# prs-eth/Marigold

Measured on AMD Instinct MI355X. Metric: depth maps/sec @768x768, ens=10, 10 DDIM steps, higher is better.
Workload: dtype bf16; 1 GPU; marigold-depth-v1-1 architecture (SD-v2 UNet 865.9M + AutoencoderKL), 768x768, ensemble_size=10, 10 DDIM steps (trailing, zero-SNR, v-prediction), seeded synthetic weights; members_per_gpu=10, parallelism=member-parallel x1, hipgraph=False, maps_in_flight=2

## Files before the change

include/marigold_hip.h:

```cpp
#ifndef MARIGOLD_HIP_H
#define MARIGOLD_HIP_H

#include <stdint.h>

#ifdef __cplusplus
extern "C" {
#endif

#define MG_ABI_VERSION 4

enum mg_op_kind {
  MG_OP_IGEMM = 1,
  MG_OP_GN_STATS = 2,
  MG_OP_GN_FINALIZE = 3,
  MG_OP_GN_APPLY = 4,
  MG_OP_GN_SLAB = 9,
  MG_OP_ROWGEMM = 10,
  MG_OP_FLASH_ATTN64 = 6,
  MG_OP_FLASH_ATTN512 = 11,
  MG_OP_SOFTMAX_ROWS = 7,
  MG_OP_SCHED_STEP = 12,
  MG_OP_LINEAR_SMALL_M = 13,
  MG_OP_LATENT_1X1 = 14,
  MG_OP_POST_NCHW = 15,
// ... 675 lines not shown
  const float* conv_b[5];
  const float* lin_w[5];
} mg_lpips_net;
long long mg_lpips_workspace_bytes(int H, int W);
int mg_eval_iid_lpips(const mg_lpips_net* net, const float* pred, const float* gt, const uint8_t* mask_or_null, int H, int W,
                      int up_to_scale, int gamma_mode, double* out8, void* eval_ws, void* act_ws, long long act_ws_bytes, void* stream);

int mg_rgb_prepare(const uint8_t* src, int hwc, int Hin, int Win, void* dst, int out16, int Hout, int Wout, int mode, int reciprocal,
                   float* tmp_or_null, void* stream);
int mg_normals_visualize(const float* pred, int H, int W, uint8_t* out_hwc, void* stream);
int mg_depth_visualize(const float* depth, const uint8_t* lut256x3_or_null, int64_t n, float* clipped_out_or_null,
                       uint16_t* u16_out_or_null, uint8_t* picture_out_or_null, void* stream);
int mg_normals_finish(const float* pred, int H, int W, float* clipped_out_or_null, uint8_t* picture_out_or_null, void* stream);

int mg_randn(uint64_t seed, uint64_t stream_id, int64_t offset, int64_t n, void* dst, int out16, void* stream);
int mg_resize(const void* src, void* dst, float* tmp_or_null, int planes, int Hin, int Win, int Hout, int Wout, int mode, int u8,
              void* stream);
int mg_colorize(const float* depth, const uint8_t* lut256x3, uint8_t* out_hwc, int64_t n, float min_depth, float max_depth, void* stream);
int mg_iid_visualize(const float* pred, uint8_t* out_hwc, float* workspace_or_null, int n_targets, int H, int W, int linear_bits,
                     int up_to_scale_bits, void* stream);

int mg_ens_align_cost_grad(int E, const double* s, const double* t, const double* mean, const double* C,
                           double* cost, double* gs, double* gt);
int mg_bfgs_minimize(int (*fn)(void* user, int n, const double* x, double* f, double* g), void* user, int n, double* x,
                     double gtol, int maxiter, double* fval, int* nit, int* nfev, int* status);
int mg_ens_align_minimize(const mg_op* reg_op, void* stream, int E, int affine, int reduction, double lam, const double* mean,
                          const double* C, float* st_host, const float* mm_host, double* x, double gtol, int maxiter,
                          double* fval, int* nit, int* nfev, int* status);

int mg_clock_probe(void* stream, int zero_operands, double* mhz, double* tflops);

int mg_debug_read_workspace(void* host_dst, long long bytes);

void* mg_event_create(void);
int mg_event_record(void* ev, void* stream);
int mg_event_elapsed_ms(void* start, void* stop, float* ms);
void mg_event_destroy(void* ev);

#ifdef __cplusplus
}
#endif
#endif
```

marigold_amd/_lib.py:

```python
import ctypes
import os

_HERE = os.path.dirname(os.path.abspath(__file__))
LIB_PATH = os.environ.get("MARIGOLD_HIP_LIB") or os.path.join(_HERE, "libmarigold_hip.so")
ABI_VERSION = 4

OP_IGEMM, OP_GN_STATS, OP_GN_FINALIZE, OP_GN_APPLY = 1, 2, 3, 4
OP_FLASH_ATTN64, OP_SOFTMAX_ROWS = 6, 7
OP_GN_SLAB = 9
OP_ROWGEMM = 10
OP_FLASH_ATTN512 = 11
RG_BF16, RG_GEGLU, RG_QKV, RG_XATTN = 0, 1, 2, 3
OP_SCHED_STEP = 12
OP_LINEAR_SMALL_M, OP_LATENT_1X1, OP_POST_NCHW, OP_IM2COL_SMALL = 13, 14, 15, 16
OP_CONV3X3 = 17
OP_CONV3X3_HEAD = 18
OP_ENS_DEPTH_STATS, OP_ENS_DEPTH_MEDIAN, OP_ENS_DEPTH_NORM, OP_ENS_NORMALS = 20, 21, 22, 23
OP_RESIZE = 24
OP_COLORIZE = 25
OP_EVAL_DEPTH_LS, OP_EVAL_DEPTH_METRICS, OP_EVAL_NORMALS = 26, 27, 28
EVAL_WS_BYTES = 128 * 1024
EVAL_ALIGN = {None: 0, "least_square": 1, "least_square_disparity": 2}
OP_MEMSET, OP_COPY = 30, 31
OP_IIDSCORE_PREP, OP_IIDSCORE_PSNR, OP_IIDSCORE_SSIM = 32, 33, 34
# ... 136 lines not shown
        p=("pred", "gt", "mask", "sums", "out", "scratch"))),
    OP_EVAL_NORMALS: ("EVAL_NORMALS", dict(
        i=("masked",),
        p=("pred", "gt", "out", "err", "ws"),
        l=("hw",))),
    OP_MEMSET: ("MEMSET", dict(
        i=("value",),
        p=("dst",),
        l=("bytes",))),
    OP_COPY: ("COPY", dict(
        p=("src", "dst"),
        l=("bytes",))),
    OP_IIDSCORE_PREP: ("IIDSCORE_PREP", dict(
        i=("h", "w", "gamma"),
        p=("pred", "gt", "mask", "out", "ws"))),
    OP_IIDSCORE_PSNR: ("IIDSCORE_PSNR", dict(
        i=("h", "w", "gamma", "up_to_scale", "write_psnr"),
        p=("pred", "gt", "mask", "out", "ws"))),
    OP_IIDSCORE_SSIM: ("IIDSCORE_SSIM", dict(
        i=("h", "w", "gamma", "up_to_scale"),
        p=("pred", "gt", "mask", "out", "ws"))),
    OP_IID_VIS: ("IID_VIS", dict(
        i=("n", "h", "w", "linear_bits", "up_to_scale_bits"),
        p=("pred", "out", "ws"))),
}

OP_NAMES = {v: k[3:].lower() for k, v in list(globals().items()) if k.startswith("OP_")}

EXPORTS = [
    "mg_abi_version", "mg_operand_bits", "mg_last_error", "mg_init", "mg_geglu_interleave", "mg_device_info", "mg_launch",
    "mg_program_create", "mg_program_num_ops", "mg_program_run", "mg_program_validate", "mg_program_run_range",
    "mg_program_capture", "mg_program_profile", "mg_program_destroy", "mg_conv2d_igemm", "mg_conv3x3", "mg_conv3x3_gn_slots", "mg_flash4w_plan_test",
    "mg_sched_step", "mg_ensemble_normals", "mg_ens_align_cost_grad", "mg_bfgs_minimize", "mg_ens_align_minimize", "mg_event_create", "mg_event_record",
    "mg_event_elapsed_ms", "mg_event_destroy", "mg_clock_probe", "mg_debug_read_workspace",
    "mg_model_load", "mg_model_destroy", "mg_model_info", "mg_model_device_bytes", "mg_model_validate", "mg_model_vae_encode",
    "mg_model_denoise", "mg_model_vae_decode", "mg_ensemble_depth", "mg_eval_depth", "mg_eval_normals", "mg_eval_iid",
    "mg_rgb_prepare", "mg_normals_visualize",
    "mg_randn", "mg_resize", "mg_colorize", "mg_iid_visualize", "mg_model_predict",
    "mg_ensemble_iid", "mg_model_predict_iid",
    "mg_depth_visualize", "mg_normals_finish", "mg_model_predict_out",
    "mg_lpips_workspace_bytes", "mg_eval_iid_lpips",
]


class MgPredictOpts(ctypes.Structure):
    _fields_ = [("scale_invariant", ctypes.c_int), ("shift_invariant", ctypes.c_int), ("reduction", ctypes.c_int), ("max_iter", ctypes.c_int),
                ("max_res", ctypes.c_int), ("normals_reduction", ctypes.c_int), ("regularizer_strength", ctypes.c_double), ("tol", ctypes.c_double)]

    def __init__(self, scale_invariant=1, shift_invariant=1, reduction=0, max_iter=50, max_res=1024, normals_reduction=0,
                 regularizer_strength=0.02, tol=1e-6):
        super().__init__(scale_invariant, shift_invariant, reduction, max_iter, max_res, normals_reduction, regularizer_strength, tol)


class MgIidOpts(ctypes.Structure):
    _fields_ = [("reduction", ctypes.c_int), ("linear_bits", ctypes.c_int), ("up_to_scale_bits", ctypes.c_int), ("out_h", ctypes.c_int),
                ("out_w", ctypes.c_int), ("out_mode", ctypes.c_int)]


class MgOutputOpts(ctypes.Structure):
    _fields_ = [("out_h", ctypes.c_int), ("out_w", ctypes.c_int), ("out_mode", ctypes.c_int), ("lut256x3", ctypes.c_void_p)]


class MgLpipsNet(ctypes.Structure):
    _fields_ = [("conv_w", ctypes.c_void_p * 5), ("conv_b", ctypes.c_void_p * 5), ("lin_w", ctypes.c_void_p * 5)]


class MgOp(ctypes.Structure):
# ... 23 lines not shown
    missing = [s for s in EXPORTS if not hasattr(lib, s)]
    if missing:
        raise MarigoldHipError(f"{path} lacks ABI symbols: {missing}")
    lib.mg_last_error.restype = ctypes.c_char_p
    lib.mg_launch.argtypes = [ctypes.POINTER(MgOp), ctypes.c_void_p]
    lib.mg_geglu_interleave.restype = ctypes.c_int
    lib.mg_conv2d_igemm.argtypes = [ctypes.POINTER(MgOp), ctypes.c_void_p]
    lib.mg_conv3x3.argtypes = [ctypes.POINTER(MgOp), ctypes.c_void_p]
    lib.mg_conv3x3_gn_slots.argtypes = [ctypes.POINTER(MgOp)]
    lib.mg_conv3x3_gn_slots.restype = ctypes.c_int
    lib.mg_flash4w_plan_test.argtypes = [ctypes.c_int] * 4 + [ctypes.c_longlong, ctypes.c_int, ctypes.POINTER(ctypes.c_int), ctypes.POINTER(ctypes.c_uint)]
    lib.mg_program_create.restype = ctypes.c_void_p
    lib.mg_program_create.argtypes = [ctypes.POINTER(MgOp), ctypes.c_int]
    lib.mg_program_num_ops.argtypes = [ctypes.c_void_p]
    lib.mg_ens_align_cost_grad.argtypes = [ctypes.c_int] + [ctypes.c_void_p] * 7
    lib.mg_bfgs_minimize.argtypes = [ctypes.c_void_p, ctypes.c_void_p, ctypes.c_int, ctypes.c_void_p, ctypes.c_double, ctypes.c_int,
                                     ctypes.c_void_p, ctypes.c_void_p, ctypes.c_void_p, ctypes.c_void_p]
    lib.mg_ens_align_minimize.argtypes = [ctypes.c_void_p, ctypes.c_void_p, ctypes.c_int, ctypes.c_int, ctypes.c_int, ctypes.c_double,
                                          ctypes.c_void_p, ctypes.c_void_p, ctypes.c_void_p, ctypes.c_void_p, ctypes.c_void_p,
                                          ctypes.c_double, ctypes.c_int, ctypes.c_void_p, ctypes.c_void_p, ctypes.c_void_p, ctypes.c_void_p]
    lib.mg_program_run.argtypes = [ctypes.c_void_p, ctypes.c_void_p]
    lib.mg_program_validate.argtypes = [ctypes.c_void_p]
    lib.mg_program_run_range.argtypes = [ctypes.c_void_p, ctypes.c_int, ctypes.c_int, ctypes.c_void_p]
    lib.mg_program_capture.argtypes = [ctypes.c_void_p, ctypes.c_void_p]
    lib.mg_program_profile.argtypes = [ctypes.c_void_p, ctypes.c_void_p, ctypes.POINTER(ctypes.c_float)]
    lib.mg_program_destroy.argtypes = [ctypes.c_void_p]
    lib.mg_program_destroy.restype = None
    lib.mg_sched_step.argtypes = [ctypes.c_void_p] * 4 + [ctypes.c_int64] + [ctypes.c_float] * 3 + [ctypes.c_void_p]
    lib.mg_ensemble_normals.argtypes = [ctypes.c_void_p] * 3 + [ctypes.c_int, ctypes.c_int64, ctypes.c_int, ctypes.c_void_p]
    lib.mg_device_info.argtypes = [ctypes.POINTER(ctypes.c_int), ctypes.POINTER(ctypes.c_int),
                                   ctypes.POINTER(ctypes.c_int64), ctypes.c_char_p, ctypes.c_int]
    lib.mg_clock_probe.argtypes = [ctypes.c_void_p, ctypes.c_int, ctypes.POINTER(ctypes.c_double), ctypes.POINTER(ctypes.c_double)]
    lib.mg_debug_read_workspace.argtypes = [ctypes.c_void_p, ctypes.c_longlong]
    lib.mg_model_load.restype = ctypes.c_void_p
    lib.mg_model_load.argtypes = [ctypes.c_char_p, ctypes.c_int]
    lib.mg_model_destroy.argtypes = [ctypes.c_void_p]
    lib.mg_model_destroy.restype = None
    lib.mg_model_info.argtypes = [ctypes.c_void_p, ctypes.POINTER(ctypes.c_int)]
    lib.mg_model_device_bytes.argtypes = [ctypes.c_void_p]
    lib.mg_model_device_bytes.restype = ctypes.c_longlong
    lib.mg_model_validate.argtypes = [ctypes.c_void_p]
    lib.mg_model_vae_encode.argtypes = [ctypes.c_void_p] * 4
    lib.mg_model_denoise.argtypes = [ctypes.c_void_p] * 5
    lib.mg_model_vae_decode.argtypes = [ctypes.c_void_p] * 4
    lib.mg_ensemble_depth.argtypes = [ctypes.c_void_p, ctypes.c_int, ctypes.c_int, ctypes.c_int, ctypes.c_int, ctypes.c_int, ctypes.c_int, ctypes.c_double,
                                      ctypes.c_int, ctypes.c_double, ctypes.c_int, ctypes.c_void_p, ctypes.c_void_p, ctypes.c_void_p, ctypes.c_void_p]
    lib.mg_eval_depth.argtypes = [ctypes.c_void_p] * 3 + [ctypes.c_int] * 4 + [ctypes.c_double] * 2 + [ctypes.c_void_p] * 3
    lib.mg_eval_normals.argtypes = [ctypes.c_void_p] * 2 + [ctypes.c_int64, ctypes.c_int] + [ctypes.c_void_p] * 4
    lib.mg_eval_iid.argtypes = [ctypes.c_void_p] * 3 + [ctypes.c_int] * 5 + [ctypes.c_void_p] * 3
    lib.mg_lpips_workspace_bytes.argtypes = [ctypes.c_int, ctypes.c_int]
    lib.mg_lpips_workspace_bytes.restype = ctypes.c_longlong
    lib.mg_eval_iid_lpips.argtypes = [ctypes.POINTER(MgLpipsNet)] + [ctypes.c_void_p] * 3 + [ctypes.c_int] * 4 + [ctypes.c_void_p] * 3 + \
        [ctypes.c_longlong, ctypes.c_void_p]
    lib.mg_rgb_prepare.argtypes = [ctypes.c_void_p] + [ctypes.c_int] * 3 + [ctypes.c_void_p] + [ctypes.c_int] * 5 + [ctypes.c_void_p] * 2
    lib.mg_normals_visualize.argtypes = [ctypes.c_void_p, ctypes.c_int, ctypes.c_int, ctypes.c_void_p, ctypes.c_void_p]
    lib.mg_randn.argtypes = [ctypes.c_uint64, ctypes.c_uint64, ctypes.c_int64, ctypes.c_int64, ctypes.c_void_p, ctypes.c_int, ctypes.c_void_p]
    lib.mg_resize.argtypes = [ctypes.c_void_p] * 3 + [ctypes.c_int] * 7 + [ctypes.c_void_p]
    lib.mg_colorize.argtypes = [ctypes.c_void_p] * 3 + [ctypes.c_int64, ctypes.c_float, ctypes.c_float, ctypes.c_void_p]
    lib.mg_iid_visualize.argtypes = [ctypes.c_void_p] * 3 + [ctypes.c_int] * 5 + [ctypes.c_void_p]
    lib.mg_model_predict.argtypes = [ctypes.c_void_p] * 2 + [ctypes.c_int] * 5 + [ctypes.c_uint64, ctypes.POINTER(MgPredictOpts)] + [ctypes.c_void_p] * 4
    lib.mg_ensemble_iid.argtypes = [ctypes.c_void_p, ctypes.c_int, ctypes.c_int64, ctypes.c_int, ctypes.c_void_p, ctypes.c_void_p, ctypes.c_void_p]
    lib.mg_model_predict_iid.argtypes = [ctypes.c_void_p] * 2 + [ctypes.c_int] * 5 + [ctypes.c_uint64, ctypes.POINTER(MgIidOpts)] + [ctypes.c_void_p] * 4
    lib.mg_depth_visualize.argtypes = [ctypes.c_void_p] * 2 + [ctypes.c_int64] + [ctypes.c_void_p] * 4
    lib.mg_normals_finish.argtypes = [ctypes.c_void_p, ctypes.c_int, ctypes.c_int] + [ctypes.c_void_p] * 3
    lib.mg_model_predict_out.argtypes = [ctypes.c_void_p] * 2 + [ctypes.c_int] * 5 + [ctypes.c_uint64, ctypes.POINTER(MgPredictOpts),
                                                                                       ctypes.POINTER(MgOutputOpts)] + [ctypes.c_void_p] * 6
# ... 31 lines not shown
```

marigold_amd/csrc/common.h:

```cpp
#pragma once
#include <hip/hip_runtime.h>
#include <stdint.h>

#include <type_traits>
#include "../../include/marigold_hip.h"

constexpr bool MG_F16 = MG_OPERAND_F16_BUILD != 0;
typedef uint16_t bf16_t;
typedef std::conditional_t<MG_F16, _Float16, __bf16> mg_op16_t;
typedef __attribute__((ext_vector_type(8))) mg_op16_t bf16x8;
typedef __attribute__((ext_vector_type(2))) mg_op16_t mg_bf16x2_t;
typedef __attribute__((ext_vector_type(2))) float mg_f32x2_t;
typedef __attribute__((ext_vector_type(16))) float f32x16;
typedef __attribute__((ext_vector_type(4))) float f32x4;

#define GLOBAL_AS __attribute__((address_space(1)))
#define LDS_AS __attribute__((address_space(3)))

#if MG_OPERAND_F16_BUILD
#define MG_MFMA32_ASM "v_mfma_f32_32x32x16_f16"
#define MG_MFMA16_ASM "v_mfma_f32_16x16x32_f16"
#define MG_CVT_PK_ASM "v_cvt_pk_f16_f32"
#else
#define MG_MFMA32_ASM "v_mfma_f32_32x32x16_bf16"
// ... 107 lines not shown
}

struct mg_fastdiv {
  uint32_t m, l;
};
inline mg_fastdiv mg_make_fastdiv(long long d) {
  mg_fastdiv f;
  uint32_t l = 0;
  while ((1ull << l) < (unsigned long long)d) ++l;
  f.l = l;
  f.m = (uint32_t)(((1ull << (31 + l)) + (unsigned long long)d - 1) / (unsigned long long)d);
  return f;
}
__device__ __forceinline__ int fdiv(int x, const mg_fastdiv f) { return (int)(__umulhi((uint32_t)x << 1, f.m) >> f.l); }

constexpr bool MG_HANDOFF_FENCES = MG_HANDOFF_FENCES_BUILD != 0;
__device__ __forceinline__ void mg_handoff_release() {
  if constexpr (MG_HANDOFF_FENCES) {
    __builtin_amdgcn_fence(__ATOMIC_RELEASE, "agent");
    asm volatile("s_waitcnt vmcnt(0)" ::: "memory");
  }
}
__device__ __forceinline__ void mg_handoff_acquire() {
  if constexpr (MG_HANDOFF_FENCES) __builtin_amdgcn_fence(__ATOMIC_ACQUIRE, "agent");
}

#define MG_ZERO_BYTES (128 * 1024)
extern void* g_zero_page;
extern thread_local bool g_dry_run;
#define MG_SPLITK_WS_BYTES (64ll * 1024 * 1024)
#define MG_LN_COUNTERS 65536
extern unsigned* g_ln_counters;
extern void* g_splitk_ws;
#define MG_LAUNCH(...)                                   \
  do {                                                   \
    if (!g_dry_run) hipLaunchKernelGGL(__VA_ARGS__);     \
  } while (0)
void mg_set_error(const char* fmt, ...);
int mg_tuning_int(const char* name, int dflt);
#define MG_CHECK_HIP(expr)                                                         \
  do {                                                                             \
    hipError_t _e = (expr);                                                        \
    if (_e != hipSuccess) {                                                        \
      mg_set_error("%s failed: %s (%s:%d)", #expr, hipGetErrorString(_e), __FILE__, __LINE__); \
      return 1;                                                                    \
    }                                                                              \
  } while (0)
int mg_kernel_max_lds(const void* kern, int bytes, bool no_static_lds = false);
#define MG_KERNEL_MAX_LDS(...)                                   \
  do {                                                           \
    if (const int _rc = mg_kernel_max_lds(__VA_ARGS__)) return _rc; \
  } while (0)
int mg_cu_count();
#define MG_REQUIRE(cond, ...)      \
  do {                             \
    if (!(cond)) {                 \
      mg_set_error(__VA_ARGS__);   \
      return 2;                    \
    }                              \
  } while (0)

int mg_launch_igemm(const mg_op* op, hipStream_t s);
int mg_launch_igemm2(const mg_op* op, hipStream_t s, int variant);
int mg_launch_conv_patch(const mg_op* op, hipStream_t s);
int mg_conv3x3_gn_slots_of(const mg_op* op);
int mg_launch_rowgemm(const mg_op* op, hipStream_t s);
// ... 10 lines not shown
```

marigold_amd/csrc/igemm2.hip:

```cpp
#include "igemm2_body.h"

void* mg_igemm2_big_kernel(int which);

namespace {

template <int BM, int BN, int WGM, int WGN, int NSTAGE, bool TRANS, bool SPLIT, bool PF, int ABL = 0, int BK = 64>
__global__ __launch_bounds__(WGM* WGN * 64) void igemm2_kernel(const Igemm2Args a) {
  igemm2_body<BM, BN, WGM, WGN, NSTAGE, TRANS, SPLIT, PF ? 1 : 0, ABL, BK>(a);
}

template <bool TRANS, int PPOPT>
__global__ __launch_bounds__(512) void igemm2_pingpong_kernel(const Igemm2Args a) {
  igemm2_body<256, 256, 2, 4, 2, TRANS, false, 2, 0, 64, PPOPT>(a);
}

__global__ __launch_bounds__(256) void splitk_reduce_kernel(const Igemm2Args a) {
  const int nv = a.N >> 3;
  const long long total = (long long)a.M * nv;
  for (long long i = (long long)blockIdx.x * 256 + threadIdx.x; i < total; i += (long long)gridDim.x * 256) {
    const int m = (int)(i / nv);
    const int n = (int)(i - (long long)m * nv) * 8;
    float v[8];
#pragma unroll
    for (int j = 0; j < 8; ++j) v[j] = 0.f;
    for (int sidx = 0; sidx < a.splits; ++sidx) {
      const float* p = a.ws + ((long long)sidx * a.M + m) * a.N + n;
      const float4 x0 = *(const float4*)p, x1 = *(const float4*)(p + 4);
      v[0] += x0.x; v[1] += x0.y; v[2] += x0.z; v[3] += x0.w;
      v[4] += x1.x; v[5] += x1.y; v[6] += x1.z; v[7] += x1.w;
    }
#pragma unroll
    for (int j = 0; j < 8; ++j) v[j] *= a.scale;
    if (a.bias) {
      const float4 b0 = *(const float4*)(a.bias + n), b1 = *(const float4*)(a.bias + n + 4);
      v[0] += b0.x; v[1] += b0.y; v[2] += b0.z; v[3] += b0.w;
      v[4] += b1.x; v[5] += b1.y; v[6] += b1.z; v[7] += b1.w;
    }
    if (a.rowvec) {
      const float* rv = a.rowvec + (long long)(m / a.rows_per_img) * a.rv_stride + n;
      const float4 r0 = *(const float4*)rv, r1 = *(const float4*)(rv + 4);
      v[0] += r0.x; v[1] += r0.y; v[2] += r0.z; v[3] += r0.w;
// ... 26 lines not shown
  b.cpt = a.Cin / BK;
  b.c0t = a.A1 ? a.C0 / BK : b.cpt;
  b.xcpt = a.xcin / BK;
  b.xc0t = a.X1 ? a.xc0 / BK : b.xcpt;
  b.KT = a.taps * b.cpt + b.xcpt;
  b.tiles_m = (a.M + BM - 1) / BM;
  b.tiles_n = (a.n_end - a.n_begin + BN - 1) / BN;
  b.splits = 1;
  b.kps = b.KT;
  b.ws = nullptr;
  const long long tiles = (long long)b.tiles_m * b.tiles_n;
  const bool sk_ok = !TRANS && a.splits >= 0 && batch_z == 1 && a.epi == MG_EPI_BF16 && a.n_begin == 0 && a.n_end == a.N && (a.ws || g_splitk_ws);
  if (sk_ok && (a.splits > 1 || (a.splits == 0 && tiles < 160 && b.KT >= 32))) {
    int sp;
    if (a.splits > 1) {
      sp = min(a.splits, max(1, b.KT / 2));
    } else {
      sp = (int)min((long long)8, (320 + tiles - 1) / tiles);
      if constexpr (BIG == 2 || BIG == 3) sp = (int)min((long long)8, max(1ll, 256 / tiles));
      sp = min(sp, b.KT / 12);
    }
    {
      static const int skmax = mg_tuning_int("MARIGOLD_SPLITK_MAX", 0);
      if (skmax > 0) sp = min(sp, skmax);
    }
    const long long per_split = (long long)a.M * a.N * 4;
    while (sp > 1 && (long long)sp * per_split > MG_SPLITK_WS_BYTES) --sp;
    if (sp > 1) {
      b.kps = (b.KT + sp - 1) / sp;
      b.splits = (b.KT + b.kps - 1) / b.kps;
      b.ws = a.ws ? a.ws : (float*)g_splitk_ws;
    }
  }
  const long long grid = tiles * b.splits * batch_z;
  MG_REQUIRE(grid > 0 && grid < (1ll << 31), "igemm: bad grid %lld", grid);
  b.fd_per_z = mg_make_fastdiv(tiles * b.splits);
  b.fd_tiles = mg_make_fastdiv(tiles);
  b.fd_tiles_n = mg_make_fastdiv(b.tiles_n);
  b.fd_cpt = mg_make_fastdiv(b.cpt);
  MG_LAUNCH(kern, dim3((unsigned)grid), dim3(NT), LDS, s, b);
  if (b.splits > 1) {
    const long long nvec = (long long)a.M * (a.N / 8);
    MG_LAUNCH(splitk_reduce_kernel, dim3((unsigned)min((nvec + 255) / 256, (long long)4096)), dim3(256), 0, s, b);
  }
  if (!g_dry_run) MG_CHECK_HIP(hipGetLastError());
  return 0;
}

template <bool TRANS>
int dispatch_tile(const Igemm2Args& a, int batch_z, int variant, hipStream_t s) {
  switch (variant) {
    case 22: return launch2<128, 128, 4, 2, 3, TRANS>(a, batch_z, s);
    case 23: return launch2<64, 64, 2, 2, 2, TRANS>(a, batch_z, s);
    case 24: return launch2<64, 64, 2, 2, 4, TRANS>(a, batch_z, s);
    case 25: return launch2<128, 64, 2, 2, 4, TRANS, true>(a, batch_z, s);
    case 26: return launch2<128, 128, 2, 2, 3, TRANS, true>(a, batch_z, s);
    case 29: return launch2<128, 32, 4, 1, 3, TRANS>(a, batch_z, s);
    case 54: return launch2<128, 64, 4, 1, 3, TRANS, true>(a, batch_z, s);
    case 32: return launch2<128, 128, 2, 2, 2, TRANS, true>(a, batch_z, s);
    case 35: return launch2<128, 64, 2, 2, 3, TRANS, true>(a, batch_z, s);
    case 36: return launch2<256, 128, 4, 2, 3, TRANS, true, true>(a, batch_z, s);
    case 51: return launch2<256, 128, 2, 2, 3, TRANS, true, false, 0, 32>(a, batch_z, s);
    case 62: return launch2<256, 256, 2, 4, 2, TRANS, false, false, 0, 64, 4>(a, batch_z, s);
    case 72:
      if constexpr (!TRANS) {
        MG_REQUIRE((long long)(a.M / a.rows_per_img) * a.H * a.W * max(max(a.lda, a.lda1), max(a.ldx0, a.ldx1)) < (1ll << 30) && (long long)a.N * a.ldw < (1ll << 30),
                   "igemm: tile variant 72 addresses its operands with 31-bit byte offsets");
        return launch2<256, 256, 2, 2, 2, false, false, false, 0, 64, -1, 2>(a, batch_z, s);
      } else MG_REQUIRE(false, "igemm: tile variant 72 has no transposed section");
      return 0;
    case 73:
      if constexpr (!TRANS) {
        MG_REQUIRE((long long)(a.M / a.rows_per_img) * a.H * a.W * max(max(a.lda, a.lda1), max(a.ldx0, a.ldx1)) < (1ll << 30) && (long long)a.N * a.ldw < (1ll << 30),
                   "igemm: tile variant 73 addresses its operands with 31-bit byte offsets");
// ... 217 lines not shown
```

marigold_amd/csrc/igemm2_big.hip:

```cpp
#include "igemm2_body.h"

namespace {

__global__ __launch_bounds__(256) __attribute__((amdgpu_waves_per_eu(1, 1))) void igemm2_k4w_kernel(const Igemm2Args a) {
  igemm2_body<256, 256, 2, 2, 2, false, false, 3, 0, 64>(a);
}

__global__ __launch_bounds__(256) __attribute__((amdgpu_waves_per_eu(1, 1))) void igemm2_k4wb_kernel(const Igemm2Args a) {
  igemm2_body<192, 320, 2, 2, 2, false, false, 3, 0, 64>(a);
}

__global__ __launch_bounds__(256) __attribute__((amdgpu_waves_per_eu(1, 1))) void igemm2_k4w_stamped_kernel(const Igemm2Args a) {
  igemm2_body<256, 256, 2, 2, 2, false, false, 3, 0, 64, 0, true>(a);
}
__global__ __launch_bounds__(256) __attribute__((amdgpu_waves_per_eu(1, 1))) void igemm2_k4wb_stamped_kernel(const Igemm2Args a) {
  igemm2_body<192, 320, 2, 2, 2, false, false, 3, 0, 64, 0, true>(a);
}

}

void* mg_igemm2_big_kernel(int which) {
  if (which >= 4) return which == 5 ? (void*)igemm2_k4wb_stamped_kernel : (void*)igemm2_k4w_stamped_kernel;
  return which == 3 ? (void*)igemm2_k4wb_kernel : (void*)igemm2_k4w_kernel;
}
```

marigold_amd/csrc/igemm2_body.h:

```cpp
#pragma once
#include <stdlib.h>

#include <type_traits>

#include "common.h"
#include "igemm2_k4w.inc"

namespace {

struct Igemm2Args {
  const bf16_t* A;
  const bf16_t* A1;
  int C0, lda1, c0t;
  const bf16_t* X0;
  const bf16_t* X1;
  int xcin, xc0, ldx0, ldx1, xcpt, xc0t;
  const bf16_t* Wt;
  void* out;
  const float* bias;
  const float* rowvec;
  const bf16_t* res;
  const void* zero;
  int H, W, Cin, Ho, Wo, N, taps, stride, pad, Hu, Wu, epi, ldo, ldr, lda, ldt, ldw;
  int tw;
  int subpix;
  int M, rows_per_img, tiles_m, tiles_n, cpt, KT, rv_stride, up2, ctr;
  int n_begin, n_end;
  int splits, kps;
  float* ws;
  long long sA, sW, sO, sR;
  float scale;
  const float2* ln_in;
  const float* ln_g;
  const float* ln_c;
  float2* ln_out;
  unsigned* ln_ctr;
  float ln_eps;
  float sm_scale;
  int sm_cols;
  mg_fastdiv fd_per_z, fd_tiles, fd_tiles_n, fd_rpi, fd_wo, fd_cpt;
  int lin;
  double inv_n;
  int tperm;
  const bf16_t* w2;
  unsigned long long* stamps;
  int c2;
  double inv_c2;
};

__device__ __forceinline__ uint32_t cvt_pk_bf16(float lo, float hi) { return cvt_pk_bf16_f32(lo, hi); }

template <int N>
__device__ __forceinline__ void wait_vmcnt() {
  asm volatile("s_waitcnt vmcnt(%0)" ::"n"(N) : "memory");
}

template <int BM, int BN, int WGM, int WGN, int NSTAGE, bool TRANS, bool SPLIT, int LOOP, int ABL, int BK, int PPOPT = 0, bool STAMP = false>
__device__ __forceinline__ void igemm2_body(const Igemm2Args& a) {
  constexpr bool PF = LOOP == 1, PP = LOOP == 2, K4 = LOOP == 3;
  static_assert(!K4 || (((BM == 256 && BN == 256) || (BM == 192 && BN == 320)) && WGM == 2 && WGN == 2 && NSTAGE == 2 && BK == 64 &&
                        ABL == 0 && !TRANS),
                "the hand-placed one-wave-per-SIMD schedule is written for the 256x256 and 192x320 / 4-wave / 2-buffer tiles");
  static_assert(!PP || (BM == 256 && BN == 256 && WGM == 2 && WGN == 4 && NSTAGE == 2 && BK == 64 && ABL == 0),
                "the ping-pong schedule is written for the 256x256 / 8-wave / 2-stage tile");
  constexpr int NT = WGM * WGN * 64;
  constexpr int TM = BM / WGM, TN = BN / WGN, MI = TM / 32, NI = TN / 32;
  constexpr int ROWB = BK * 2;
  constexpr int CPR = BK / 8;
  constexpr int KS = BK / 16;
  constexpr int A_IT = BM * CPR / NT, B_IT = BN * CPR / NT;
  constexpr int LOADS = A_IT + B_IT;
  constexpr int STAGE = (BM + BN) * ROWB;
  static_assert(BK == 64 || BK == 32, "BK is 64 or 32");
  static_assert((BM * CPR) % NT == 0 && (BN * CPR) % NT == 0, "every thread stages a whole number of 16-byte chunks");
  auto swz = [](int chunk, int r) { return BK == 64 ? (chunk ^ ((r >> 1) & 7)) : (chunk ^ ((r >> 2) & 3)); };
  constexpr int D = NSTAGE - 1;
  static_assert(A_IT >= 1 && B_IT >= 1 && MI >= 1 && NI >= 1, "tile too small for the block");
  static_assert(NSTAGE >= 2 && NSTAGE <= 4, "2..4 LDS stages");
  extern __shared__ __attribute__((aligned(16))) char smem[];

  const int tid = threadIdx.x;
  const int lane = tid & 63;
  const int wave = __builtin_amdgcn_readfirstlane(tid >> 6);
  const int wm = wave / WGN, wn = wave % WGN;
  const int l31 = lane & 31, half = lane >> 5;

  const int bid = xcd_remap(blockIdx.x, gridDim.x);
  auto stamp = [&](int k) {
    if constexpr (STAMP) {
      if (a.stamps && tid == 0) a.stamps[(long long)blockIdx.x * 8 + k] = __builtin_amdgcn_s_memrealtime();
// ... 598 lines not shown
        for (int idx = 0; idx < LOADS; idx += 2) issue_piece(st_i, idx);
      }
      mfmas(fa0[1], fb0[1]);
      if constexpr (ISSUE) {
#pragma unroll
        for (int idx = 1; idx < LOADS; idx += 2) issue_piece(st_i, idx);
        advance();
      }
      __builtin_amdgcn_sched_barrier(0);
      if constexpr (NEXT) {
        asm volatile("s_waitcnt lgkmcnt(0)" ::: "memory");
        if constexpr (ISSUE) wait_vmcnt<LOADS>();
        else wait_vmcnt<0>();
        __builtin_amdgcn_s_barrier();
        const char* sN = smem + st_n * STAGE;
        load_frags(sN, 0, fa0[0], fb0[0]);
        load_frags(sN, 1, fa0[1], fb0[1]);
      }
      __builtin_amdgcn_sched_barrier(0);
      mfmas(fa1[0], fb1[0]);
      mfmas(fa1[1], fb1[1]);
      __builtin_amdgcn_sched_barrier(0);
      st_c = (st_c + 1 == NSTAGE) ? 0 : st_c + 1;
      st_n = (st_n + 1 == NSTAGE) ? 0 : st_n + 1;
      st_i = (st_i + 1 == NSTAGE) ? 0 : st_i + 1;
    };
    int kt = 0;
    for (; kt + 2 < KT; ++kt) k_step(std::true_type{}, std::true_type{});
    for (; kt + 1 < KT; ++kt) k_step(std::false_type{}, std::true_type{});
    for (; kt < KT; ++kt) k_step(std::false_type{}, std::false_type{});
  }

  stamp(3);
  const float scale = a.scale;
  const float* const zf = (const float*)a.zero;
  auto store_slot = [&](float2* p, float s2, float q2) {
    const unsigned long long bits = ((unsigned long long)__float_as_uint(q2) << 32) | __float_as_uint(s2);
    __hip_atomic_store((unsigned long long*)p, bits, __ATOMIC_RELAXED, __HIP_MEMORY_SCOPE_AGENT);
  };
  auto ln_out_finish = [&]() {
    asm volatile("s_waitcnt vmcnt(0)" ::: "memory");
    __syncthreads();
    int* const flag = (int*)smem;
    if (tid == 0) {
      mg_handoff_release();
      const unsigned ticket = __hip_atomic_fetch_add(&a.ln_ctr[tile_m], 1u, __ATOMIC_RELAXED, __HIP_MEMORY_SCOPE_AGENT);
      const bool last = ticket == (unsigned)(a.tiles_n - 1);
      if (last) {
        mg_handoff_acquire();
        __hip_atomic_store(&a.ln_ctr[tile_m], 0u, __ATOMIC_RELAXED, __HIP_MEMORY_SCOPE_AGENT);
      }
      *flag = last ? 1 : 0;
    }
    __syncthreads();
    if (*flag == 0) return;
    const int slots = a.N >> 5;
    float2* const mr = a.ln_out + (long long)a.M * slots;
    static_assert(BM % (NT / 8) == 0, "whole passes of NT / 8 rows");
    for (int r = tid >> 3; r < BM; r += NT >> 3) {
      const int m = m0 + r, sub = tid & 7;
      double sd = 0.0, qd = 0.0;
      if (m < a.M) {
        const unsigned long long* p = (const unsigned long long*)(a.ln_out + (long long)m * slots);
        for (int sl0 = sub; sl0 < slots; sl0 += 40) {
          unsigned long long v[5];
#pragma unroll
// ... 543 lines not shown
```

marigold_amd/csrc/runtime.hip:

```cpp
#include <stdarg.h>
#include <stdio.h>
#include <stdlib.h>
#include <string.h>

#include <atomic>
#include <mutex>
#include <vector>

#include "common.h"
#include "kernel_once.h"

void* g_zero_page = nullptr;
void* g_splitk_ws = nullptr;
unsigned* g_ln_counters = nullptr;
thread_local bool g_dry_run = false;
static thread_local char g_err[512] = "";
static std::mutex g_init_mutex;
static int g_device = -1;
static std::atomic<int> g_cu_count{256};
static mg_kernel_once g_kernel_once;

int mg_cu_count() { return g_cu_count.load(std::memory_order_relaxed); }

int mg_kernel_max_lds(const void* kern, int bytes, bool no_static_lds) {
  return g_kernel_once.raise(kern, bytes, g_dry_run, [no_static_lds](const void* k, int b) {
    if (no_static_lds) {
      hipFuncAttributes fa;
      MG_CHECK_HIP(hipFuncGetAttributes(&fa, k));
      MG_REQUIRE(fa.sharedSizeBytes == 0, "this kernel's dynamic LDS must start at LDS address 0 (static LDS %d bytes)", (int)fa.sharedSizeBytes);
    }
    MG_CHECK_HIP(hipFuncSetAttribute(k, hipFuncAttributeMaxDynamicSharedMemorySize, b));
    return 0;
  });
}

int mg_tuning_int(const char* name, int dflt) {
  static const bool on = [] { const char* e = getenv("MARIGOLD_TUNING"); return e && e[0] == '1'; }();
  if (!on) return dflt;
  const char* e = getenv(name);
  return e && e[0] ? atoi(e) : dflt;
}

void mg_set_error(const char* fmt, ...) {
  va_list ap;
  va_start(ap, fmt);
  vsnprintf(g_err, sizeof(g_err), fmt, ap);
  va_end(ap);
}

struct mg_program {
  std::vector<mg_op> ops;
  hipGraph_t graph = nullptr;
  hipGraphExec_t exec = nullptr;
};

static int dispatch(const mg_op* op, hipStream_t s) {
  switch (op->kind) {
    case MG_OP_IGEMM: return mg_launch_igemm(op, s);
    case MG_OP_CONV3X3: return mg_launch_conv_patch(op, s);
    case MG_OP_ROWGEMM: return mg_launch_rowgemm(op, s);
    case MG_OP_GN_STATS:
    case MG_OP_GN_FINALIZE:
    case MG_OP_GN_APPLY:
    case MG_OP_GN_SLAB: return mg_launch_norm(op, s);
    case MG_OP_FLASH_ATTN512: return mg_launch_flash512(op, s);
    case MG_OP_FLASH_ATTN64:
// ... 315 lines not shown
  MG_CHECK_HIP(hipDeviceGetAttribute(&cus, hipDeviceAttributeMultiprocessorCount, dev));
  const hipStream_t s = (hipStream_t)stream;
  ClockProbeRes R;
  MG_CHECK_HIP(hipMalloc(&R.d_out, (size_t)(2 * cus + 1) * 8));
  MG_CHECK_HIP(hipMalloc(&R.d_data, 512 * 16));
  unsigned h[2048];
  unsigned seed = 12345u;
  for (int i = 0; i < 2048; ++i) {
    seed = seed * 1664525u + 1013904223u;
    const unsigned lo = 0x3f00u | ((seed >> 8) & 0x80ffu), hi = 0x3f00u | ((seed >> 20) & 0x80ffu);
    h[i] = zero_operands ? 0u : (lo | (hi << 16));
  }
  MG_CHECK_HIP(hipMemcpyAsync(R.d_data, h, sizeof(h), hipMemcpyHostToDevice, s));
  const int iters = 20000;
  MG_CHECK_HIP(hipEventCreate(&R.e0));
  MG_CHECK_HIP(hipEventCreate(&R.e1));
  float ms = 0.f;
  for (int rep = 0; rep < 2; ++rep) {
    MG_CHECK_HIP(hipEventRecord(R.e0, s));
    hipLaunchKernelGGL(clock_probe_kernel, dim3(cus), dim3(256), 0, s, R.d_out, R.d_data, iters);
    MG_CHECK_HIP(hipEventRecord(R.e1, s));
    MG_CHECK_HIP(hipStreamSynchronize(s));
  }
  MG_CHECK_HIP(hipEventElapsedTime(&ms, R.e0, R.e1));
  std::vector<unsigned long long> r(2 * cus);
  MG_CHECK_HIP(hipMemcpy(r.data(), R.d_out, (size_t)2 * cus * 8, hipMemcpyDeviceToHost));
  double sc = 0.0, rt = 0.0;
  for (int i = 0; i < cus; ++i) { sc += (double)r[2 * i]; rt += (double)r[2 * i + 1]; }
  *mhz = rt > 0.0 ? sc / rt * 100.0 : 0.0;
  *tflops = ms > 0.f ? (double)cus * 4.0 * iters * 8.0 * 2.0 * 32 * 32 * 16 / (ms * 1e-3) / 1e12 : 0.0;
  return 0;
}

int mg_debug_read_workspace(void* host_dst, long long bytes) {
  MG_REQUIRE(host_dst && bytes > 0 && bytes <= MG_SPLITK_WS_BYTES && g_splitk_ws, "mg_debug_read_workspace: bad arguments");
  MG_CHECK_HIP(hipDeviceSynchronize());
  MG_CHECK_HIP(hipMemcpy(host_dst, g_splitk_ws, (size_t)bytes, hipMemcpyDeviceToHost));
  return 0;
}

void* mg_event_create(void) {
  hipEvent_t e = nullptr;
  if (hipEventCreate(&e) != hipSuccess) return nullptr;
  return (void*)e;
}
int mg_event_record(void* ev, void* stream) {
  MG_CHECK_HIP(hipEventRecord((hipEvent_t)ev, (hipStream_t)stream));
  return 0;
}
int mg_event_elapsed_ms(void* start, void* stop, float* ms) {
  MG_CHECK_HIP(hipEventSynchronize((hipEvent_t)stop));
  MG_CHECK_HIP(hipEventElapsedTime(ms, (hipEvent_t)start, (hipEvent_t)stop));
  return 0;
}
void mg_event_destroy(void* ev) {
  if (ev) hipEventDestroy((hipEvent_t)ev);
}

}
```

Before: 3.798 depth maps/s.

## Fuse split-K reduction into the igemm launch via per-tile tickets

Split-K igemm launches now write per-split partial tiles to a workspace slab and take an atomic ticket per output tile. The last split to arrive sums the other slabs into its accumulators and runs the bf16 epilogue itself, so the separate splitk_reduce kernel launch and its full re-read of the workspace are no longer needed. This adds an atomic handoff, a serial tail on the last-arriving workgroup, lazily allocated ticket buffers that cannot be allocated during graph capture, and a tuning flag to disable the path.

```diff
diff --git a/include/marigold_hip.h b/include/marigold_hip.h
--- a/include/marigold_hip.h
+++ b/include/marigold_hip.h
@@ -731,6 +731,8 @@
 
 int mg_debug_read_workspace(void* host_dst, long long bytes);
 
+int mg_debug_read_splitk_tickets(const void* ws, unsigned* host_dst, int n);
+
 void* mg_event_create(void);
 int mg_event_record(void* ev, void* stream);
 int mg_event_elapsed_ms(void* start, void* stop, float* ms);
diff --git a/marigold_amd/_lib.py b/marigold_amd/_lib.py
--- a/marigold_amd/_lib.py
+++ b/marigold_amd/_lib.py
@@ -192,7 +192,7 @@
     "mg_program_create", "mg_program_num_ops", "mg_program_run", "mg_program_validate", "mg_program_run_range",
     "mg_program_capture", "mg_program_profile", "mg_program_destroy", "mg_conv2d_igemm", "mg_conv3x3", "mg_conv3x3_gn_slots", "mg_flash4w_plan_test",
     "mg_sched_step", "mg_ensemble_normals", "mg_ens_align_cost_grad", "mg_bfgs_minimize", "mg_ens_align_minimize", "mg_event_create", "mg_event_record",
-    "mg_event_elapsed_ms", "mg_event_destroy", "mg_clock_probe", "mg_debug_read_workspace",
+    "mg_event_elapsed_ms", "mg_event_destroy", "mg_clock_probe", "mg_debug_read_workspace", "mg_debug_read_splitk_tickets",
     "mg_model_load", "mg_model_destroy", "mg_model_info", "mg_model_device_bytes", "mg_model_validate", "mg_model_vae_encode",
     "mg_model_denoise", "mg_model_vae_decode", "mg_ensemble_depth", "mg_eval_depth", "mg_eval_normals", "mg_eval_iid",
     "mg_rgb_prepare", "mg_normals_visualize",
@@ -282,6 +282,7 @@
                                    ctypes.POINTER(ctypes.c_int64), ctypes.c_char_p, ctypes.c_int]
     lib.mg_clock_probe.argtypes = [ctypes.c_void_p, ctypes.c_int, ctypes.POINTER(ctypes.c_double), ctypes.POINTER(ctypes.c_double)]
     lib.mg_debug_read_workspace.argtypes = [ctypes.c_void_p, ctypes.c_longlong]
+    lib.mg_debug_read_splitk_tickets.argtypes = [ctypes.c_void_p, ctypes.c_void_p, ctypes.c_int]
     lib.mg_model_load.restype = ctypes.c_void_p
     lib.mg_model_load.argtypes = [ctypes.c_char_p, ctypes.c_int]
     lib.mg_model_destroy.argtypes = [ctypes.c_void_p]
diff --git a/marigold_amd/csrc/common.h b/marigold_amd/csrc/common.h
--- a/marigold_amd/csrc/common.h
+++ b/marigold_amd/csrc/common.h
@@ -163,6 +163,9 @@
 #define MG_LN_COUNTERS 65536
 extern unsigned* g_ln_counters;
 extern void* g_splitk_ws;
+#define MG_SPLITK_TICKETS 16384
+#define MG_SPLITK_FUSE_MAX 8
+int mg_splitk_tickets(const void* ws, hipStream_t s, unsigned** ctr);
 #define MG_LAUNCH(...)                                   \
   do {                                                   \
     if (!g_dry_run) hipLaunchKernelGGL(__VA_ARGS__);     \
diff --git a/marigold_amd/csrc/igemm2.hip b/marigold_amd/csrc/igemm2.hip
--- a/marigold_amd/csrc/igemm2.hip
+++ b/marigold_amd/csrc/igemm2.hip
@@ -7,6 +7,11 @@
 template <int BM, int BN, int WGM, int WGN, int NSTAGE, bool TRANS, bool SPLIT, bool PF, int ABL = 0, int BK = 64>
 __global__ __launch_bounds__(WGM* WGN * 64) void igemm2_kernel(const Igemm2Args a) {
   igemm2_body<BM, BN, WGM, WGN, NSTAGE, TRANS, SPLIT, PF ? 1 : 0, ABL, BK>(a);
+}
+
+template <int BM, int BN, int WGM, int WGN, int NSTAGE, bool SPLIT, bool PF, int BK>
+__global__ __launch_bounds__(WGM* WGN * 64) void igemm2_fused_kernel(const Igemm2Args a) {
+  igemm2_body<BM, BN, WGM, WGN, NSTAGE, false, SPLIT, PF ? 1 : 0, 0, BK, 0, false, true>(a);
 }
 
 template <bool TRANS, int PPOPT>
@@ -99,6 +104,24 @@
       b.ws = a.ws ? a.ws : (float*)g_splitk_ws;
     }
   }
+  constexpr bool CAN_FUSE = !TRANS && PPOPT < 0 && ABL == 0;
+  constexpr int FUSE_UP_TO = BIG >= 0 ? 0
+                             : (BM == 64 && BN == 64) ? MG_SPLITK_FUSE_MAX
+                             : (BM == 128 && BN == 128 && WGM == 4 && WGN == 2) ? 4
+                             : ((BM == 128 && BN == 64 && WGM == 2 && NSTAGE == 3) || (BM == 256 && BN == 128 && PF)) ? 3
+                             : 0;
+  bool fused = false;
+  if constexpr (CAN_FUSE) {
+    const int on = mg_tuning_int("MARIGOLD_SPLITK_FUSED", 1);
+    fused = on && b.splits > 1 && b.splits <= (on == 2 ? MG_SPLITK_FUSE_MAX : FUSE_UP_TO) && tiles <= MG_SPLITK_TICKETS &&
+            tiles * b.splits * (long long)(BM * BN * 4) <= MG_SPLITK_WS_BYTES;
+    if (fused) {
+      if constexpr (BIG >= 0) kern = (void (*)(const Igemm2Args))mg_igemm2_big_kernel(BIG + 4);
+      else kern = igemm2_fused_kernel<BM, BN, WGM, WGN, NSTAGE, SPLIT, PF, BK>;
+      MG_KERNEL_MAX_LDS((const void*)kern, LDS);
+      if (const int rc = mg_splitk_tickets(b.ws, s, &b.ln_ctr)) return rc;
+    }
+  }
   const long long grid = tiles * b.splits * batch_z;
   MG_REQUIRE(grid > 0 && grid < (1ll << 31), "igemm: bad grid %lld", grid);
   b.fd_per_z = mg_make_fastdiv(tiles * b.splits);
@@ -106,7 +129,7 @@
   b.fd_tiles_n = mg_make_fastdiv(b.tiles_n);
   b.fd_cpt = mg_make_fastdiv(b.cpt);
   MG_LAUNCH(kern, dim3((unsigned)grid), dim3(NT), LDS, s, b);
-  if (b.splits > 1) {
+  if (b.splits > 1 && !fused) {
     const long long nvec = (long long)a.M * (a.N / 8);
     MG_LAUNCH(splitk_reduce_kernel, dim3((unsigned)min((nvec + 255) / 256, (long long)4096)), dim3(256), 0, s, b);
   }
diff --git a/marigold_amd/csrc/igemm2_big.hip b/marigold_amd/csrc/igemm2_big.hip
--- a/marigold_amd/csrc/igemm2_big.hip
+++ b/marigold_amd/csrc/igemm2_big.hip
@@ -17,9 +17,17 @@
   igemm2_body<192, 320, 2, 2, 2, false, false, 3, 0, 64, 0, true>(a);
 }
 
+__global__ __launch_bounds__(256) __attribute__((amdgpu_waves_per_eu(1, 1))) void igemm2_k4w_fused_kernel(const Igemm2Args a) {
+  igemm2_body<256, 256, 2, 2, 2, false, false, 3, 0, 64, 0, false, true>(a);
+}
+__global__ __launch_bounds__(256) __attribute__((amdgpu_waves_per_eu(1, 1))) void igemm2_k4wb_fused_kernel(const Igemm2Args a) {
+  igemm2_body<192, 320, 2, 2, 2, false, false, 3, 0, 64, 0, false, true>(a);
+}
+
 }
 
 void* mg_igemm2_big_kernel(int which) {
+  if (which >= 6) return which == 7 ? (void*)igemm2_k4wb_fused_kernel : (void*)igemm2_k4w_fused_kernel;
   if (which >= 4) return which == 5 ? (void*)igemm2_k4wb_stamped_kernel : (void*)igemm2_k4w_stamped_kernel;
   return which == 3 ? (void*)igemm2_k4wb_kernel : (void*)igemm2_k4w_kernel;
 }
diff --git a/marigold_amd/csrc/igemm2_body.h b/marigold_amd/csrc/igemm2_body.h
--- a/marigold_amd/csrc/igemm2_body.h
+++ b/marigold_amd/csrc/igemm2_body.h
@@ -55,7 +55,8 @@
   asm volatile("s_waitcnt vmcnt(%0)" ::"n"(N) : "memory");
 }
 
-template <int BM, int BN, int WGM, int WGN, int NSTAGE, bool TRANS, bool SPLIT, int LOOP, int ABL, int BK, int PPOPT = 0, bool STAMP = false>
+template <int BM, int BN, int WGM, int WGN, int NSTAGE, bool TRANS, bool SPLIT, int LOOP, int ABL, int BK, int PPOPT = 0, bool STAMP = false,
+          bool FUSE = false>
 __device__ __forceinline__ void igemm2_body(const Igemm2Args& a) {
   constexpr bool PF = LOOP == 1, PP = LOOP == 2, K4 = LOOP == 3;
   static_assert(!K4 || (((BM == 256 && BN == 256) || (BM == 192 && BN == 320)) && WGM == 2 && WGN == 2 && NSTAGE == 2 && BK == 64 &&
@@ -720,6 +721,176 @@
   }
 
   stamp(3);
+
+  if constexpr (FUSE) {
+    static_assert(!TRANS && !PP && !STAMP, "the in-launch split-K finish serves the plain bf16 epilogue");
+    typedef __attribute__((ext_vector_type(4))) unsigned u32x4;
+    constexpr int NF = NI * MI;
+    constexpr unsigned SLAB = (unsigned)BM * BN * 4;
+    const int splits = a.splits;
+    const int me = __builtin_amdgcn_readfirstlane(split);
+    const int tile = __builtin_amdgcn_readfirstlane(t);
+    const __amdgpu_buffer_rsrc_t wsr =
+        __builtin_amdgcn_make_buffer_rsrc((char*)a.ws + (long long)tile * splits * (long long)SLAB, 0, 0x7fffffff, 0x00020000);
+    const unsigned lane_off = (unsigned)tid * 16u;
+    {
+      const unsigned mine = (unsigned)me * SLAB + lane_off;
+#pragma unroll
+      for (int ni = 0; ni < NI; ++ni)
+#pragma unroll
+        for (int mi = 0; mi < MI; ++mi)
+#pragma unroll
+          for (int q = 0; q < 4; ++q) {
+            const u32x4 v = {__float_as_uint(acc[ni][mi][4 * q]), __float_as_uint(acc[ni][mi][4 * q + 1]),
+                             __float_as_uint(acc[ni][mi][4 * q + 2]), __float_as_uint(acc[ni][mi][4 * q + 3])};
+            __builtin_amdgcn_raw_buffer_store_b128(v, wsr, mine + (unsigned)(((ni * MI + mi) * 4 + q) * NT * 16), 0, 16);
+          }
+    }
+    asm volatile("s_waitcnt vmcnt(0)" ::: "memory");
+    __syncthreads();
+    int* const flag = (int*)smem;
+    if (tid == 0) {
+      mg_handoff_release();
+      const unsigned ticket = __hip_atomic_fetch_add(&a.ln_ctr[tile], 1u, __ATOMIC_RELAXED, __HIP_MEMORY_SCOPE_AGENT);
+      const bool last = ticket == (unsigned)(splits - 1);
+      if (last) {
+        mg_handoff_acquire();
+        __hip_atomic_store(&a.ln_ctr[tile], 0u, __ATOMIC_RELAXED, __HIP_MEMORY_SCOPE_AGENT);
+      }
+      *flag = last ? 1 : 0;
+    }
+    __syncthreads();
+    if (*flag == 0) return;
+    auto sum_slabs = [&](auto smax_tag) {
+#pragma clang fp contract(off)
+      constexpr int SMAX = decltype(smax_tag)::value;
+      constexpr int GF0 = (K4 ? 8 : 4) / (SMAX - 1);
+      constexpr int GF = GF0 < 1 ? 1 : (GF0 > NF ? NF : GF0);
+#pragma unroll
+      for (int f0 = 0; f0 < NF; f0 += GF) {
+        u32x4 P[GF][SMAX - 1][4];
+#pragma unroll
+        for (int g = 0; g < GF; ++g) {
+          if (f0 + g >= NF) break;
+#pragma unroll
+          for (int k = 0; k < SMAX - 1; ++k) {
+            if (k < splits - 1) {
+              const unsigned slab = (unsigned)(k < me ? k : k + 1) * SLAB + lane_off;
+#pragma unroll
+              for (int q = 0; q < 4; ++q)
+                P[g][k][q] = __builtin_amdgcn_raw_buffer_load_b128(wsr, slab + (unsigned)(((f0 + g) * 4 + q) * NT * 16), 0, 16);
+            }
+          }
+        }
+#pragma unroll
+        for (int g = 0; g < GF; ++g) {
+          if (f0 + g >= NF) break;
+          const int ni = (f0 + g) / MI, mi = (f0 + g) % MI;
+          f32x16 sum;
+#pragma unroll
+          for (int r = 0; r < 16; ++r) sum[r] = 0.f;
+#pragma unroll
+          for (int k = 0; k < SMAX; ++k) {
+            if (k == me) {
+#pragma unroll
+              for (int r = 0; r < 16; ++r) sum[r] += acc[ni][mi][r];
+            }
+            if (k < SMAX - 1 && k < splits - 1) {
+              const int kk = k < SMAX - 1 ? k : 0;
+#pragma unroll
+              for (int q = 0; q < 4; ++q) {
+                sum[4 * q] += __uint_as_float(P[g][kk][q].x); sum[4 * q + 1] += __uint_as_float(P[g][kk][q].y);
+                sum[4 * q + 2] += __uint_as_float(P[g][kk][q].z); sum[4 * q + 3] += __uint_as_float(P[g][kk][q].w);
+              }
+            }
+          }
+          acc[ni][mi] = sum;
+        }
+      }
+    };
+    if (splits <= 2) sum_slabs(std::integral_constant<int, 2>{});
+    else if (splits <= 4) sum_slabs(std::integral_constant<int, 4>{});
+    else sum_slabs(std::integral_constant<int, 8>{});
+    auto epilogue = [&](auto rv_tag, auto res_tag) {
+#pragma clang fp contract(off)
+      constexpr bool RV = decltype(rv_tag)::value, RES = decltype(res_tag)::value;
+      constexpr int PER = 2 + (RV ? 2 * MI : 0) + (RES ? MI : 0);
+      constexpr int BUDGET = NT >= 512 ? 16 : (K4 ? 48 : 24);
+      constexpr int EB = BUDGET / PER < 1 ? 1 : (BUDGET / PER > 2 * NI ? 2 * NI : BUDGET / PER);
+      const bool has_b = a.bias != nullptr;
+      int e_m[MI], e_img[MI];
+#pragma unroll
+      for (int mi = 0; mi < MI; ++mi) {
+        const int m = m0 + wm * TM + mi * 32 + l31;
+        e_m[mi] = m < a.M ? m : a.M - 1;
+        e_img[mi] = RV ? fdiv(e_m[mi], a.fd_rpi) : 0;
+      }
+#pragma unroll
+      for (int blk0 = 0; blk0 < 2 * NI; blk0 += EB) {
+        float4 xb[EB][2], xrv[EB][RV ? MI : 1][2];
+        uint4 xr[EB][RES ? MI : 1];
+#pragma unroll
+        for (int e = 0; e < EB; ++e) {
+          if (blk0 + e >= 2 * NI) break;
+          const int n = n0 + wn * TN + (blk0 + e) * 16 + 8 * half;
+          const int nc = n < a.n_end ? n : n0;
+          if (has_b) { xb[e][0] = *(const float4*)(a.bias + nc); xb[e][1] = *(const float4*)(a.bias + nc + 4); }
+#pragma unroll
+          for (int mi = 0; mi < MI; ++mi) {
+            if constexpr (RV) {
+              const float* rv = a.rowvec + (long long)e_img[mi] * a.rv_stride + nc;
+              xrv[e][mi][0] = *(const float4*)rv;
+              xrv[e][mi][1] = *(const float4*)(rv + 4);
+            }
+            if constexpr (RES) xr[e][mi] = *(const uint4*)(a.res + (long long)e_m[mi] * a.ldr + nc);
+          }
+        }
+#pragma unroll
+        for (int e = 0; e < EB; ++e) {
+          if (blk0 + e >= 2 * NI) break;
+          const int ni = (blk0 + e) >> 1, gp = (blk0 + e) & 1;
+          const int n = n0 + wn * TN + (blk0 + e) * 16 + 8 * half;
+          const bool nok = n < a.n_end;
+#pragma unroll
+          for (int mi = 0; mi < MI; ++mi) {
+            float v[8];
+#pragma unroll
+            for (int j = 0; j < 4; ++j) half_swap(acc[ni][mi][8 * gp + j], acc[ni][mi][8 * gp + 4 + j], v[j], v[4 + j]);
+#pragma unroll
+            for (int j = 0; j < 8; ++j) v[j] *= a.scale;
+            if (has_b) {
+              v[0] += xb[e][0].x; v[1] += xb[e][0].y; v[2] += xb[e][0].z; v[3] += xb[e][0].w;
+              v[4] += xb[e][1].x; v[5] += xb[e][1].y; v[6] += xb[e][1].z; v[7] += xb[e][1].w;
+            }
+            if constexpr (RV) {
+              v[0] += xrv[e][mi][0].x; v[1] += xrv[e][mi][0].y; v[2] += xrv[e][mi][0].z; v[3] += xrv[e][mi][0].w;
+              v[4] += xrv[e][mi][1].x; v[5] += xrv[e][mi][1].y; v[6] += xrv[e][mi][1].z; v[7] += xrv[e][mi][1].w;
+            }
+            if constexpr (RES) {
+              const uint4 r4 = xr[e][mi];
+              v[0] += bflo(r4.x); v[1] += bfhi(r4.x); v[2] += bflo(r4.y); v[3] += bfhi(r4.y);
+              v[4] += bflo(r4.z); v[5] += bfhi(r4.z); v[6] += bflo(r4.w); v[7] += bfhi(r4.w);
+            }
+            uint4 pk;
+            pk.x = cvt_pk_bf16(v[0], v[1]); pk.y = cvt_pk_bf16(v[2], v[3]);
+            pk.z = cvt_pk_bf16(v[4], v[5]); pk.w = cvt_pk_bf16(v[6], v[7]);
+            const int m = m0 + wm * TM + mi * 32 + l31;
+            if (m < a.M && nok) *(uint4*)((bf16_t*)a.out + (long long)m * a.ldo + n) = pk;
+          }
+        }
+      }
+    };
+    {
+      using T = std::true_type;
+      using F = std::false_type;
+      const bool has_rv = a.rowvec != nullptr, has_r = a.res != nullptr;
+      if (has_rv && has_r) epilogue(T{}, T{});
+      else if (has_rv) epilogue(T{}, F{});
+      else if (has_r) epilogue(F{}, T{});
+      else epilogue(F{}, F{});
+    }
+    return;
+  }
   const float scale = a.scale;
   const float* const zf = (const float*)a.zero;
   auto store_slot = [&](float2* p, float s2, float q2) {
diff --git a/marigold_amd/csrc/runtime.hip b/marigold_amd/csrc/runtime.hip
--- a/marigold_amd/csrc/runtime.hip
+++ b/marigold_amd/csrc/runtime.hip
@@ -5,6 +5,7 @@
 
 #include <atomic>
 #include <mutex>
+#include <unordered_map>
 #include <vector>
 
 #include "common.h"
@@ -32,6 +33,32 @@
     MG_CHECK_HIP(hipFuncSetAttribute(k, hipFuncAttributeMaxDynamicSharedMemorySize, b));
     return 0;
   });
+}
+
+static std::mutex g_tickets_mutex;
+static std::unordered_map<const void*, unsigned*> g_tickets;
+int mg_splitk_tickets(const void* ws, hipStream_t s, unsigned** ctr) {
+  *ctr = nullptr;
+  if (g_dry_run) return 0;
+  std::lock_guard<std::mutex> lk(g_tickets_mutex);
+  const auto it = g_tickets.find(ws);
+  if (it != g_tickets.end()) {
+    *ctr = it->second;
+    return 0;
+  }
+  hipStreamCaptureStatus cs = hipStreamCaptureStatusNone;
+  MG_CHECK_HIP(hipStreamIsCapturing(s, &cs));
+  MG_REQUIRE(cs == hipStreamCaptureStatusNone, "igemm: the first split-K launch on a workspace allocates its tickets and cannot be captured - run the program once eagerly first");
+  unsigned* p = nullptr;
+  MG_CHECK_HIP(hipMalloc((void**)&p, MG_SPLITK_TICKETS * sizeof(unsigned)));
+  if (const hipError_t e = hipMemsetAsync(p, 0, MG_SPLITK_TICKETS * sizeof(unsigned), s); e != hipSuccess) {
+    hipFree(p);
+    mg_set_error("hipMemsetAsync (split-K tickets) failed: %s", hipGetErrorString(e));
+    return 1;
+  }
+  g_tickets[ws] = p;
+  *ctr = p;
+  return 0;
 }
 
 int mg_tuning_int(const char* name, int dflt) {
@@ -413,6 +440,20 @@
   return 0;
 }
 
+int mg_debug_read_splitk_tickets(const void* ws, unsigned* host_dst, int n) {
+  MG_REQUIRE(host_dst && n > 0 && n <= MG_SPLITK_TICKETS, "mg_debug_read_splitk_tickets: bad arguments");
+  unsigned* p = nullptr;
+  {
+    std::lock_guard<std::mutex> lk(g_tickets_mutex);
+    const auto it = g_tickets.find(ws ? ws : g_splitk_ws);
+    if (it != g_tickets.end()) p = it->second;
+  }
+  MG_REQUIRE(p, "mg_debug_read_splitk_tickets: no split-K launch has finished its tiles in the launch on this workspace yet");
+  MG_CHECK_HIP(hipDeviceSynchronize());
+  MG_CHECK_HIP(hipMemcpy(host_dst, p, (size_t)n * sizeof(unsigned), hipMemcpyDeviceToHost));
+  return 0;
+}
+
 int mg_debug_read_workspace(void* host_dst, long long bytes) {
   MG_REQUIRE(host_dst && bytes > 0 && bytes <= MG_SPLITK_WS_BYTES && g_splitk_ws, "mg_debug_read_workspace: bad arguments");
   MG_CHECK_HIP(hipDeviceSynchronize());
```

New measurement: 3.804 depth maps/s (median of 4 runs). About the same (+0.2%).
